# sadPororo/AD-YOLO

Measured on AMD Instinct MI355X. Metric: train-step audio-sec/s (4ch, se-resnet34+adyolo), higher is better.
Workload: dtype f32

## Files before the change

### ad-yolo_amd/_lib.py

```python
import ctypes
import os

_HERE = os.path.dirname(os.path.abspath(__file__))
LIB_PATH = os.environ.get("ADYOLO_LIB") or os.path.join(_HERE, "libadyolo_hip.so")

P = ctypes.c_void_p
I = ctypes.c_int
L = ctypes.c_long
F = ctypes.c_float
U64 = ctypes.c_uint64

SIGNATURES = {
    "adyolo_abi_version": (I, []),
    "adyolo_last_error": (ctypes.c_char_p, []),
    "adyolo_feat_stft_mel": (I, [P] * 8 + [I, I] + [P] * 4 + [I, I, I, P]),
    "adyolo_feat_finish": (I, [P] * 4 + [I, I, I, P]),
    "adyolo_feat_gcc_phat": (I, [P] * 6 + [I, I, I, I, P]),
    "adyolo_nchw_to_nhwc8": (I, [P, P, I, I, I, I, P]),
    "adyolo_pack_w3x3": (I, [P, P, P, I, I, I, P]),
    "adyolo_conv3x3_tiles": (I, [I] * 3),
    "adyolo_conv3x3_fwd": (I, [P] * 13 + [I] * 7 + [P]),
    "adyolo_wino_pack_w": (I, [P, P, P, I, I, I, P]),
    "adyolo_wino_pack_many": (I, [P, I, I, I, P]),
    "adyolo_wino_tiles": (I, [I] * 3),
    "adyolo_wino_fwd": (I, [P] * 13 + [I] * 7 + [P]),
    "adyolo_wino4_pack_w": (I, [P, P, P, I, I, I, P]),
    "adyolo_wino4_pack_many": (I, [P, I, I, I, P]),
    "adyolo_wino4_tiles": (I, [I] * 3),
    "adyolo_wino4_fwd": (I, [P] * 13 + [I] * 7 + [P]),
    "adyolo_wino4_last_form": (I, []),
    "adyolo_reload_switches": (I, []),
    "adyolo_wino4_wgrad_slabs": (I, [I] * 5),
    "adyolo_wino4_wgrad": (I, [P] * 7 + [I] * 6 + [P]),
    "adyolo_wino_wgrad_slabs": (I, [I] * 5),
    "adyolo_wino_wgrad": (I, [P] * 7 + [I] * 6 + [P]),
    "adyolo_conv3x3_wgrad_slabs": (I, [I] * 5),
    "adyolo_conv3x3_wgrad": (I, [P] * 6 + [I] * 6 + [P]),
    "adyolo_gemm": (I, [P] * 5 + [I] * 10 + [P]),
    "adyolo_gemm_batched": (I, [P] * 3 + [I] * 10 + [L] * 6 + [F, I, P]),
    "adyolo_colsum": (I, [P, P, P, I, I, I, I, P]),
    "adyolo_bn_stats": (I, [P] * 7 + [I, I, I, F, F, P]),
    "adyolo_bn_stats_tiles": (I, [P] * 11 + [I, I, I, I, F, F, P]),
    "adyolo_bn_eval_stats": (I, [P] * 4 + [I, F, P]),
    "adyolo_bn_scale_shift": (I, [P] * 6 + [I, P]),
    "adyolo_affine_nhwc": (I, [P] * 4 + [L, I, P]),
    "adyolo_bn_bwd_reduce": (I, [P] * 7 + [L, I, P]),
    "adyolo_bn_bwd_tiles": (I, [P, P, P, P, I, I, P]),
    "adyolo_bn_bwd_apply": (I, [P] * 12 + [L, I, I, F, P]),
# ... 120 lines not shown
```

### ad-yolo_amd/csrc/common.hpp

```cpp
#pragma once
#include <hip/hip_runtime.h>
#include <stdint.h>
#include <stdio.h>
#include "../../include/adyolo_hip.h"

typedef float f32x16 __attribute__((ext_vector_type(16)));
typedef float f32x4 __attribute__((ext_vector_type(4)));

namespace adyolo {

void set_error(const char *fmt, ...);

inline hipStream_t as_stream(void *s) { return reinterpret_cast<hipStream_t>(s); }

inline int check_launch(const char *what) {
    hipError_t e = hipGetLastError();
    if (e != hipSuccess) {
        set_error("%s: %s", what, hipGetErrorString(e));
        return (int)e;
    }
    return 0;
}

#define ADYOLO_REQUIRE(cond, code, ...)      \
// ... 26 lines not shown

__device__ __forceinline__ void mask_bits4(const unsigned long long *__restrict__ mask, size_t i, bool &x, bool &y,
                                           bool &z, bool &w) {
    const ulonglong2 lo = *reinterpret_cast<const ulonglong2 *>(mask + (i >> 6) * 4);
    const ulonglong2 hi = *reinterpret_cast<const ulonglong2 *>(mask + (i >> 6) * 4 + 2);
    const int b = (int)(i & 63);
    x = (lo.x >> b) & 1ull; y = (lo.y >> b) & 1ull; z = (hi.x >> b) & 1ull; w = (hi.y >> b) & 1ull;
}

__device__ __forceinline__ bool mask_bit1(const unsigned long long *__restrict__ mask, size_t o) {
    const size_t i = o >> 2;
    return (mask[(i >> 6) * 4 + (o & 3)] >> (i & 63)) & 1ull;
}

__device__ __forceinline__ float sigmoidf_(float x) { return 1.0f / (1.0f + expf(-x)); }

__device__ __forceinline__ double block_colsum32(const float *__restrict__ partial, int nparts, size_t ld, int c0,
                                                 int C, double *red) {
    const int cx = threadIdx.x & 31, py = threadIdx.x >> 5;
    const int c = c0 + cx;
    double s = 0.0;
    if (c < C) {
        double s1 = 0.0, s2 = 0.0, s3 = 0.0;
        int p = py;
        for (; p + 24 < nparts; p += 32) {
            const float a0 = partial[(size_t)p * ld + c], a1 = partial[(size_t)(p + 8) * ld + c];
            const float a2 = partial[(size_t)(p + 16) * ld + c], a3 = partial[(size_t)(p + 24) * ld + c];
            s += (double)a0;
            s1 += (double)a1;
            s2 += (double)a2;
// ... 55 lines not shown
```

### ad-yolo_amd/csrc/norm.hip

```cpp
#include "common.hpp"

namespace adyolo {

#ifndef ADYOLO_EW_NT
#define ADYOLO_EW_NT 3
#endif
__device__ __forceinline__ float4 ew_ld(const float4 *p) {
#if ADYOLO_EW_NT & 1
    const f32x4 v = __builtin_nontemporal_load(reinterpret_cast<const f32x4 *>(p));
    return make_float4(v[0], v[1], v[2], v[3]);
#else
    return *p;
#endif
}
__device__ __forceinline__ void ew_st(float4 *p, const float4 &v) {
#if ADYOLO_EW_NT & 2
    const f32x4 t = {v.x, v.y, v.z, v.w};
    __builtin_nontemporal_store(t, reinterpret_cast<f32x4 *>(p));
#else
    *p = v;
#endif
}


// ... 183 lines not shown

#ifndef ADYOLO_EW_U
#define ADYOLO_EW_U 4
#endif
constexpr int EW_U = ADYOLO_EW_U;


template <bool INV>
__global__ __launch_bounds__(256) void bn_bwd_apply_kernel(
    const float *__restrict__ dy, const float *__restrict__ x, const float *__restrict__ gamma,
    const float *__restrict__ mean, const float *__restrict__ invstd, const float *__restrict__ sdy,
    const float *__restrict__ sdyx, float *__restrict__ dx, float *__restrict__ sum_partial, long n4, int c4n, float invR,
    int relu_mask) {
    __shared__ float4 sred[256];
    float4 sacc = make_float4(0.f, 0.f, 0.f, 0.f);
    float4 g, m, is, a, b;
    auto load_params = [&](int cx) {
        g = reinterpret_cast<const float4 *>(gamma)[cx];
        m = reinterpret_cast<const float4 *>(mean)[cx];
        is = reinterpret_cast<const float4 *>(invstd)[cx];
        a = reinterpret_cast<const float4 *>(sdy)[cx];
        b = reinterpret_cast<const float4 *>(sdyx)[cx];
    };
    auto one = [&](float4 d, float4 xv) {
        float4 o;
        o.x = g.x * is.x * (d.x - a.x * invR - (xv.x - m.x) * is.x * b.x * invR);
        o.y = g.y * is.y * (d.y - a.y * invR - (xv.y - m.y) * is.y * b.y * invR);
        o.z = g.z * is.z * (d.z - a.z * invR - (xv.z - m.z) * is.z * b.z * invR);
        o.w = g.w * is.w * (d.w - a.w * invR - (xv.w - m.w) * is.w * b.w * invR);
        if (relu_mask) {
            if (!(xv.x > 0.f)) o.x = 0.f;
            if (!(xv.y > 0.f)) o.y = 0.f;
            if (!(xv.z > 0.f)) o.z = 0.f;
            if (!(xv.w > 0.f)) o.w = 0.f;
        }
        sacc.x += o.x; sacc.y += o.y; sacc.z += o.z; sacc.w += o.w;
        return o;
    };
    const float4 *dy4 = reinterpret_cast<const float4 *>(dy), *x4 = reinterpret_cast<const float4 *>(x);
    float4 *dx4 = reinterpret_cast<float4 *>(dx);
    if (INV) {
        load_params((int)threadIdx.x % c4n);
        const long step = (long)gridDim.x * 256 * EW_U;
        for (long i0 = (long)blockIdx.x * 256 * EW_U + threadIdx.x; i0 < n4; i0 += step) {
            float4 d[EW_U], xv[EW_U];
#pragma unroll
            for (int u = 0; u < EW_U; ++u) {
                const long i = i0 + u * 256;
                if (i < n4) {
                    d[u] = ew_ld(&dy4[i]);
// ... 736 lines not shown
```

### ad-yolo_amd/csrc/wino4w.hip

```cpp
#include "wino4_common.hpp"

namespace adyolo {
namespace w4 {

#ifndef W4W_WHATIF
#define W4W_WHATIF 0
#endif
#ifndef W4W_LD_AUX
#define W4W_LD_AUX 0
#endif
#ifndef W4W_TIMING
#define W4W_TIMING 0
#endif

__device__ __forceinline__ void a6v(const f32x4 (&v)[4], f32x4 (&t)[6]) {
    auto fm = [](float k, f32x4 a, f32x4 b) { return pkfma4(k, a, b); };
    const f32x4 z = {0.f, 0.f, 0.f, 0.f};
    const f32x4 ea = fm(A2, v[2], v[0]), oa = fm(A3, v[3], fm(PA, v[1], z));
    const f32x4 eb = fm(B2, v[2], v[0]), ob = fm(B3, v[3], fm(PB, v[1], z));
    t[0] = v[0];
    t[1] = ea + oa;
    t[2] = fm(-1.f, oa, ea);
    t[3] = eb + ob;
    t[4] = fm(-1.f, ob, eb);
// ... 12 lines not shown
#if W4W_TIMING
__device__ unsigned long long *g_w4w_stamps;
#endif

constexpr int XROWB = 1024;
constexpr int XSLOTS = 10;
constexpr int XNU = XSLOTS * XROWB;
constexpr int XBYTES = 6 * XNU;
template <int NB>
struct DCfg {
    static constexpr int DROWB = 1024 * NB;
    static constexpr int DNU = 4 * DROWB;
    static constexpr int DBUF = 6 * DNU;
};

template <bool AFF, int NB>
__global__ __launch_bounds__(256, 1) void wino4_wgrad_kernel(
    const float *__restrict__ x, const float *__restrict__ dy, const float *__restrict__ in_scale,
    const float *__restrict__ in_shift, float *__restrict__ slabs, int N, int H, int W, int Cin, int Cout, int runsW, int npairs,
    int nseg, int seg_steps, int nitems, int nsplit, int ciBlocks, int nblk) {
    constexpr int DROWB = DCfg<NB>::DROWB, DNU = DCfg<NB>::DNU, DBUF = DCfg<NB>::DBUF;
    constexpr int XOFF = 2 * DBUF;
    __shared__ __attribute__((aligned(16))) float lds[(XBYTES + 2 * DBUF) / 4 + (AFF ? 64 : 0)];
    char *ldsb = reinterpret_cast<char *>(lds);
    constexpr int AFFOFF = XBYTES + 2 * DBUF;

    const int tid = threadIdx.x, lane = tid & 63;
    const int wave = __builtin_amdgcn_readfirstlane(tid >> 6);
    const int li = lane & 31, lh = lane >> 5;
#if W4W_TIMING
    unsigned long long *stamps = g_w4w_stamps;
    int tstep = 0;
    auto tstamp = [&](int k) {
        if (blockIdx.x == 8 && tid == 0 && tstep < 12) stamps[tstep * 16 + k] = __builtin_amdgcn_s_memtime();
    };
#else
    auto tstamp = [&](int) {};
#endif
    int split, blk;
    if (32 % nblk == 0 && (int)gridDim.x == 8 * 32) {
// ... 20 lines not shown
    f32x16 acc[9][NB];
#pragma unroll
    for (int s = 0; s < 9; ++s)
#pragma unroll
        for (int cb = 0; cb < NB; ++cb)
#pragma unroll
            for (int r = 0; r < 16; ++r) acc[s][cb][r] = 0.f;

    const int run = wave & 1;
    const int sxr = (wave >> 1) * 2 + lh, sdr = sxr;
    const int st = li >> 3, sq = li & 7;
    if (AFF) {
        if (tid < 32) lds[AFFOFF / 4 + tid] = in_scale[c0 + tid];
        else if (tid < 64) lds[AFFOFF / 4 + tid] = in_shift[c0 + tid - 32];
    }
    const int xrowb = W * Cin * 4, drowb = W * Cout * 4, xpixb = Cin * 4, dpixb = Cout * 4;
    const __amdgpu_buffer_rsrc_t xrs = __builtin_amdgcn_make_buffer_rsrc(const_cast<float *>(x), 0, (int)((size_t)N * H * W * Cin * 4), 0x00020000);
    const __amdgpu_buffer_rsrc_t drs = __builtin_amdgcn_make_buffer_rsrc(const_cast<float *>(dy), 0, (int)((size_t)N * H * W * Cout * 4), 0x00020000);
    int wl[4];
#pragma unroll
    for (int k = 0; k < 4; ++k) wl[k] = (4 * sq + ((k + sq) & 3)) * 32 + ((run ^ ((sq >> 1) & 1)) << 4) + st * 4;

    for (int item = split; item < nitems; item += nsplit) {
        const int seg = item % nseg;
        const int pair = item / nseg;
        const int q = 2 * pair + run;
        const int tW = runsW < 0 ? -runsW : 0;
        bool qok, offL, offR;
        int n, col0;
        if (tW) {
            const int sh = tW == 1 ? 0 : 1;
            n = q * (4 >> sh) + (st >> sh);
            const int tcol = st & (tW - 1);
// ... 43 lines not shown
#pragma unroll
                for (int i = 1; i < 5; ++i) xpx[i] = pkfma4v(xpx[i], xsc, shv);
                xpx[5] = pkfma4v(xpx[5], xsc, offR ? zero : shv);
            }
            bt6v(xpx);
        };
        int wx[4];
        auto x_wr2 = [&](int nu) {
#pragma unroll
            for (int k = 0; k < 4; ++k) {
                *reinterpret_cast<float *>(ldsb + wx[k] + nu * XNU) = xpx[nu][k];
                *reinterpret_cast<float *>(ldsb + wx[k] + (nu + 1) * XNU) = xpx[nu + 1][k];
            }
        };
        f32x4 dpx[NB][4], de, dq;
        const int dlane = qok ? (int)(dbase + (unsigned)sdr * (unsigned)drowb) : (int)0x80000000;
        auto d_load = [&](int trow, int cb0 = 0, int cb1 = NB, int i0 = 0, int i1 = 4) {
            const int srow = __builtin_amdgcn_readfirstlane(4 * trow * drowb);
#pragma unroll
            for (int cb = cb0; cb < cb1; ++cb)
#pragma unroll
                for (int i = i0; i < i1; ++i)
                    dpx[cb][i] = __builtin_bit_cast(f32x4, __builtin_amdgcn_raw_buffer_load_b128(drs, dlane, srow + cb * 128 + i * dpixb, W4W_LD_AUX));
        };
        int wd[4];
        auto d_put2 = [&](int cb, int nu, const f32x4 &v, const f32x4 &v1) {
#pragma unroll
            for (int k = 0; k < 4; ++k) {
                *reinterpret_cast<float *>(ldsb + wd[k] + cb * 1024 + nu * DNU) = v[k];
                *reinterpret_cast<float *>(ldsb + wd[k] + cb * 1024 + (nu + 1) * DNU) = v1[k];
            }
        };
        auto d_part = [&](int cb, int part) {
            auto fm = [](float k, f32x4 a_, f32x4 b_) { return pkfma4(k, a_, b_); };
            const f32x4 z = {0.f, 0.f, 0.f, 0.f};
            const f32x4(&v)[4] = dpx[cb];
            if (part == 0) {
                de = fm(A2, v[2], v[0]);
// ... 17 lines not shown
        for (int k = 0; k < 4; ++k) wx[k] = wl[k] + XOFF + sxr * XROWB;
#pragma unroll
        for (int nu = 0; nu < 6; nu += 2) x_wr2(nu);
        if (sxr < 2) {
            x_load(4 * t0 + 3 + sxr);
            x_prep(4 * t0 + 3 + sxr);
#pragma unroll
            for (int k = 0; k < 4; ++k) wx[k] = wl[k] + XOFF + (4 + sxr) * XROWB;
#pragma unroll
            for (int nu = 0; nu < 6; nu += 2) x_wr2(nu);
        }
#pragma unroll
        for (int k = 0; k < 4; ++k) wd[k] = wl[k] + sdr * DROWB;
#pragma unroll
        for (int cb = 0; cb < NB; ++cb) {
            d_part(cb, 0);
            d_part(cb, 1);
            d_part(cb, 2);
        }
        x_load(4 * (t0 + 1) + 1 + sxr);
        d_load(t0 + 1);
        __syncthreads();

        f32x4 a[9], b[9];
        f32x4 vF[4], vH[4], zH;
        f32x4 cF[6], cP[4], cZ[3];
        auto d_reads_full = [&](int buf_, int cb) {
            const char *dp = ldsb + buf_ * DBUF + cb * 1024 + lx;
#pragma unroll
            for (int i = 0; i < 4; ++i) vF[i] = *reinterpret_cast<const f32x4 *>(dp + nuF * DNU + i * DROWB);
// ... 52 lines not shown
            d_reads_half(buf_, 0);
        };
        auto top_xform = [&]() {
            bt6v2(cF, a[0], a[1], a[2], a[3], a[4], a[5]);
            d_xform_full();
        };
        top_full(std::integral_constant<int, 0>{}, 0);
        top_half(std::integral_constant<int, 0>{}, 0);
        top_xform();
        auto step = [&](auto ROT_, int k) {
            constexpr int rot = decltype(ROT_)::value;
            constexpr std::integral_constant<int, (rot + 4) % XSLOTS> rotn{};
            asm volatile("" : "+s"(k));
            const int buf = k & 1;
            const int gyn = 4 * (t0 + k + 1) + 1 + sxr;
            auto side = [&](int t) {
                const int gy2 = 4 * (t0 + k + 2) + 1 + sxr, tr2 = min(t0 + k + 2, H / 4 - 1);
                if (t == 1) {
                    bt3v(cP, cZ, a[6], a[7], a[8], K2x, KPx);
                    d_xform_half();
                }
                if (NB == 2) {
                    if ((W4W_WHATIF & 2) && t != 1 && t != 8 && t != 10 && t < 14) return;
                    if (t == 2) x_prep(gyn);
                    if (t >= 3 && t <= 5) x_wr2(2 * (t - 3));
                    if (t >= 4 && t <= 6) x_load(gy2, 2 * (t - 4), 2 * (t - 4) + 2);
                    if (t >= 6 && t <= 8) d_part(0, t - 6);
                    if (t == 8) {
                        d_reads_full(buf, 1);
                        d_reads_half(buf, 1);
                    }
                    if (t == 9) d_load(tr2, 0, 1, 0, 2);
                    if (t == 10) {
                        d_xform_half();
                        d_load(tr2, 0, 1, 2, 4);
                    }
                    if (t >= 11 && t <= 13) d_part(1, t - 11);
                    if (t == 14) __syncthreads();
                    if (t == 15) {
                        top_full(rotn, buf ^ 1);
                        d_load(tr2, 1, 2, 0, 2);
                    }
                    if (t == 16) {
                        top_xform();
                        d_load(tr2, 1, 2, 2, 4);
                    }
                    if (t == 17) top_half(rotn, buf ^ 1);
                } else {
                    if (t == 0) x_prep(gyn);
                    if (t >= 1 && t <= 3) x_wr2(2 * (t - 1));
                    if (t >= 2 && t <= 4) x_load(gy2, 2 * (t - 2), 2 * (t - 2) + 2);
                    if (t >= 3 && t <= 5) d_part(0, t - 3);
                    if (t == 5) d_load(tr2);
                    if (t == 6) {
                        __syncthreads();
                        top_full(rotn, buf ^ 1);
                    }
                    if (t == 7) top_xform();
                    if (t == 8) top_half(rotn, buf ^ 1);
                }
            };
            tstamp(0);
            {
                constexpr int base = (rot + 6) % XSLOTS;
                const int soff = ((base + 2 >= XSLOTS && wave >= 2) ? (base - XSLOTS) * XROWB : base * XROWB) + XOFF + sxr * XROWB;
#pragma unroll
// ... 142 lines not shown
using namespace adyolo;

#if W4W_TIMING
extern "C" int adyolo_w4w_timing_buffer(void *p) {
    return hipMemcpyToSymbol(HIP_SYMBOL(w4::g_w4w_stamps), &p, sizeof(p)) == hipSuccess ? 0 : -1;
}
#endif

extern "C" int adyolo_wino4_wgrad_slabs(int N, int H, int W, int Cin, int Cout) {
    if (N <= 0 || H <= 0 || W <= 0 || Cin <= 0 || Cout <= 0) return ADYOLO_EINVAL;
    if (Cin % 32 || Cout % 32 || (W % 16 && W != 4 && W != 8) || H % 4 || H < 8) return 0;
    if ((size_t)N * H * W * (size_t)(Cin > Cout ? Cin : Cout) * 4 >= ((size_t)1 << 31)) return 0;
    return w4::wino4_wgrad_geometry(N, H, W, Cin, Cout, nullptr, nullptr, nullptr, nullptr, nullptr);
}

extern "C" int adyolo_wino4_wgrad(const float *x, const float *dy, const float *in_scale, const float *in_shift, float *slabs,
                                  float *du, float *dw, int N, int H, int W, int Cin, int Cin_real, int Cout, void *stream) {
    ADYOLO_REQUIRE(x && dy && slabs && du && dw && N > 0 && H > 0 && W > 0, ADYOLO_EINVAL, "wino4_wgrad: bad arguments");
    ADYOLO_REQUIRE(adyolo_wino4_wgrad_slabs(N, H, W, Cin, Cout) > 0 && Cin_real > 0 && Cin_real <= Cin, ADYOLO_ENOSUP,
                   "wino4_wgrad: unsupported shape N=%d H=%d W=%d Cin=%d Cout=%d (needs Cin %% 32 == 0, Cout %% 32 == 0, W %% 16 == 0 or W = 4 | 8, "
                   "H %% 4 == 0, tensors below 2 GiB)", N, H, W, Cin, Cout);
    ADYOLO_REQUIRE((in_scale == nullptr) == (in_shift == nullptr), ADYOLO_EINVAL, "wino4_wgrad: in_scale/in_shift come together");
    ADYOLO_REQUIRE(((reinterpret_cast<size_t>(x) | reinterpret_cast<size_t>(dy) | reinterpret_cast<size_t>(in_scale) |
                     reinterpret_cast<size_t>(in_shift)) & 15) == 0, ADYOLO_ENOSUP, "wino4_wgrad: x, dy, in_scale, in_shift must be 16-byte aligned");
    hipStream_t st = as_stream(stream);
    int npairs, nseg, seg_steps, nitems, nblk;
    const int nsplit = w4::wino4_wgrad_geometry(N, H, W, Cin, Cout, &npairs, &nseg, &seg_steps, &nitems, &nblk);
    const unsigned grid = (unsigned)(nsplit * nblk);
#define ADYOLO_W4W(AFF_, NB_)                                                                                          \
    hipLaunchKernelGGL((w4::wino4_wgrad_kernel<AFF_, NB_>), dim3(grid), dim3(256), 0, st, x, dy, in_scale, in_shift, slabs, N, H, \
                       W, Cin, Cout, W >= 16 ? W / 16 : -(W / 4), npairs, nseg, seg_steps, nitems, nsplit, Cin / 32, nblk)
    if (Cout % 64 == 0) {
        if (in_scale) ADYOLO_W4W(true, 2); else ADYOLO_W4W(false, 2);
    } else {
        if (in_scale) ADYOLO_W4W(true, 1); else ADYOLO_W4W(false, 1);
    }
#undef ADYOLO_W4W
    int rc = check_launch("wino4_wgrad");
    if (rc) return rc;
    hipLaunchKernelGGL(w4::wino4_wgrad_reduce_kernel, dim3(cdiv(Cin * Cout, 32), 36), dim3(256), 0, st, slabs, du, nsplit, Cin * Cout);
    rc = check_launch("wino4_wgrad_reduce");
    if (rc) return rc;
    hipLaunchKernelGGL(w4::wino4_wgrad_finish_kernel, dim3(cdiv(Cin * Cout, 256)), dim3(256), 0, st, du, dw, Cin, Cin_real, Cout);
    return check_launch("wino4_wgrad_finish");
}
```

### ad-yolo_amd/functional.py

```python
import os
from typing import NamedTuple

import torch

from . import ops

FUSE_BNBWD = os.environ.get("ADYOLO_FUSE_BNBWD", "1") != "0"
FUSE_POOL = os.environ.get("ADYOLO_FUSE_POOL", "1") != "0"
FUSE_POOL_BWD = os.environ.get("ADYOLO_FUSE_POOL_BWD", "1") != "0"


class BlockLink:

    def __init__(self):
        self.cc = self.mean2 = self.invstd2 = self.tiles = self.ebits = None
        self.affine = self.stem_bn = None
        self.prepooled = None


class BlockArgs(NamedTuple):
    bn1: object
    bn2: object
    bnd: object = None
    link_in: object = None
# ... 299 lines not shown
        vg1, vb1 = SINK.view(pg1), SINK.view(pb1)
        sunk = vse is not None and vw1 is not None and vw2 is not None and vg1 is not None and vb1 is not None
        if not sunk:
            vse = vw1 = vw2 = vg1 = vb1 = None
        de_full = None
        if pooled_hw is not None and not ctx.has_down:
            de_full = torch.empty(n, pooled_hw[0], pooled_hw[1], c, dtype=torch.float32, device=de.device)
        dc, dr, dg2, db2, dfw1, dfb1, dfw2, dfb2 = ops.se_tail_bwd(de, e, cc, g2, b2, mean2, invstd2, ssum2, pooled,
                                                                   hid, s, fw1, fw2,
                                                                   want_dr=ctx.has_down, tile_stats=tiles,
                                                                   mask=ebits, packed_out=vse, pooled_hw=pooled_hw,
                                                                   de_out=de_full)
        if pooled_hw is not None:
            de = de_full
        dw2 = ops.conv3x3_wgrad(a, dc, c, in_affine=(scale1, shift1), out=vw2)
        if FUSE_BNBWD:
            dbb, st = ops.conv3x3(dc, wpk2d, c, want_stats=True, stat_bn=(a, mean1, invstd1))
            da, dg1, db1 = ops.bn_bwd(dbb, a, g1, mean1, invstd1, relu_mask=True, tile_stats=st, out_dgamma=vg1,
                                      out_dbeta=vb1)
        else:
            dbb = ops.conv3x3(dc, wpk2d, c)
            da, dg1, db1 = ops.bn_bwd(dbb, a, g1, mean1, invstd1, relu_mask=True, out_dgamma=vg1, out_dbeta=vb1)
        dw1 = ops.conv3x3_wgrad(p, da, cin, in_affine=ctx.p_aff, out=vw1)
        if sunk:
            SINK.done(*pse)
            SINK.done(pw2, pg1, pb1, pw1)
            dw1 = dg1 = db1 = dw2 = dg2 = db2 = dfw1 = dfb1 = dfw2 = dfb2 = None
        dwd = dgd = dbd = None
        if ctx.has_down:
            q, wd, gd, meand, invstdd = t[20:25]
            pwd, pgd, pbd, wdshape = ctx.down_ptrs
            vwd, vgd, vbd = SINK.view(pwd, (wdshape[0], wdshape[1])), SINK.view(pgd), SINK.view(pbd)
            dsunk = sunk and vwd is not None and vgd is not None and vbd is not None
            if not dsunk:
                vwd = vgd = vbd = None
            dq, dgd, dbd = ops.bn_bwd(dr, q, gd, meand, invstdd, relu_mask=False, out_dgamma=vgd, out_dbeta=vbd)
            rows = n * h * w_
            dwd = ops.gemm(dq, p, c, cin, rows, c, cin, trans_a=True, trans_b=True,
# ... 535 lines not shown
```

### ad-yolo_amd/ops.py

```python
import ctypes
import os

import numpy as np
import torch

from . import _lib

_c = _lib.call
NULL = ctypes.c_void_p(0)


def _p(t):
    if t is None:
        return NULL
    return ctypes.c_void_p(t.data_ptr())


def _stream():
    return ctypes.c_void_p(torch.cuda.current_stream().cuda_stream)


def _chk(*ts):
    for t in ts:
        if t is None:
# ... 102 lines not shown

W4_THRESHOLDS = {}
_THRESHOLD_KEYS = ("min_k", "min_k_addend", "min_wgs", "min_wgrad_work", "min_k_32")


def reload_thresholds():
    env = os.environ.get
    W4_THRESHOLDS.update(min_k=int(env("ADYOLO_W4_MIN_K", "32")),
                         min_k_addend=int(env("ADYOLO_W4_MIN_K_ADDEND", "32")),
                         min_wgs=int(env("ADYOLO_W4_MIN_WGS", "200")),
                         min_wgrad_work=int(env("ADYOLO_W4W_MIN_WORK", "6000000")),
                         min_k_32=int(env("ADYOLO_W4_MIN_K_32", "32")),
                         persist=env("ADYOLO_W4_PERSIST", "1") != "0",
                         narrow=env("ADYOLO_W4_NARROW", "1") != "0",
                         wino1d=env("ADYOLO_WINO1D", "1") != "0",
                         wgrad_algo=(env("ADYOLO_WGRAD_ALGO") or "").lower() or None)
    if _lib.loaded():
        _lib.load().adyolo_reload_switches()
    return {k: W4_THRESHOLDS[k] for k in _THRESHOLD_KEYS}


def switch_table():
    t = dict(W4_THRESHOLDS)
    t["conv_algo"] = conv_algo()
    return t


def switch_stamp():
    return tuple(sorted((k, str(v)) for k, v in switch_table().items()))


# ... 151 lines not shown
    return (y, stats) if want_stats else y


def wgrad_form(cin, cout, algo=None, shape=None):
    algo = algo or W4_THRESHOLDS["wgrad_algo"] or conv_algo()
    if algo == "winograd4" and shape is not None and cin % 32 == 0 and cout % 32 == 0:
        n, h, w = shape
        if (w % 16 == 0 or w in (4, 8)) and h % 4 == 0 and n * w // 16 * (h // 4) * cin * cout >= W4_THRESHOLDS["min_wgrad_work"] and \
                _lib.load().adyolo_wino4_wgrad_slabs(n, h, w, cin, cout) > 0:
            return "wino4_wgrad_kernel", 9.0 / 36.0
    if algo in ("winograd", "winograd4") and cin % 32 == 0 and cout % 32 == 0:
        return "wino_wgrad_kernel", 16.0 / 36.0
    return "conv3x3_wgrad_kernel", 1.0


def conv3x3_wgrad(x, dy, cin_real, in_affine=None, algo=None, out=None):
    _chk(x, dy)
    n, h, w, cin = x.shape
    cout = dy.shape[3]
    sc, sh = in_affine if in_affine is not None else (None, None)
    dw = out if out is not None else _new(x, cout, cin_real, 3, 3)
    form = wgrad_form(cin, cout, algo, (n, h, w))[0]
    if DISPATCH_LOG is not None:
        k = (form, cin, cout, 1 if in_affine is not None else 0)
        DISPATCH_LOG[k] = DISPATCH_LOG.get(k, 0) + 1
    if form == "wino4_wgrad_kernel":
        nslab = _lib.load().adyolo_wino4_wgrad_slabs(n, h, w, cin, cout)
        slabs = _new(x, nslab, 36, cin, cout)
        du = _new(x, 36, cin, cout)
        _c("adyolo_wino4_wgrad", _p(x), _p(dy), _p(sc), _p(sh), _p(slabs), _p(du), _p(dw), n, h, w, cin, cin_real, cout, _stream())
# ... 140 lines not shown


def affine(x, scale, shift):
    _chk(x, scale, shift)
    c = x.shape[-1]
    y = torch.empty_like(x)
    _c("adyolo_affine_nhwc", _p(x), _p(scale), _p(shift), _p(y), x.numel() // c, c, _stream())
    return y


def bn_bwd(dy, x, gamma, mean, invstd, relu_mask=False, tile_stats=None, out_dgamma=None, out_dbeta=None,
           want_dx_colsum=False):
    _chk(dy, x, gamma, mean, invstd)
    c = x.shape[-1]
    rows = x.numel() // c
    sdy = out_dbeta if out_dbeta is not None else _new(x, c)
    sdyx = out_dgamma if out_dgamma is not None else _new(x, c)
    if tile_stats is not None:
        _c("adyolo_bn_bwd_tiles", _p(tile_stats), _p(sdy), _p(sdyx), _p(_new(tile_stats, 2, 256, c)), tile_stats.shape[1], c,
           _stream())
    else:
        partial = _new(x, 2 * 1024 * c)
        _c("adyolo_bn_bwd_reduce", _p(dy), _p(x), _p(mean), _p(invstd), _p(sdy), _p(sdyx), _p(partial), rows, c,
           _stream())
    dx = torch.empty_like(x)
    colsum = part = None
    if want_dx_colsum:
        colsum, part = _new(x, c), _new(x, 8192, c)
    a_sdy, a_sdyx, cs = sdy, sdyx, 1.0
    if EXACT.on:
        glob = EXACT.all_reduce(torch.stack([sdy, sdyx]))
        a_sdy, a_sdyx, cs = glob[0], glob[1], float(EXACT.world)
    _c("adyolo_bn_bwd_apply", _p(dy), _p(x), _p(gamma), _p(mean), _p(invstd), _p(a_sdy), _p(a_sdyx), _p(dx), NULL, NULL,
       _p(colsum), _p(part), rows, c, int(relu_mask), cs, _stream())
    if want_dx_colsum:
        return dx, sdyx, sdy, colsum
    return dx, sdyx, sdy


def se_fc_fwd(ssum, scale, shift, w1, b1, w2, b2, hw):
    _chk(ssum, scale, shift, w1, b1, w2, b2)
    n, c = ssum.shape
    cr = w1.shape[0]
    pooled, hid, s = _new(ssum, n, c), _new(ssum, n, cr), _new(ssum, n, c)
    _c("adyolo_se_fc_fwd", _p(ssum), _p(scale), _p(shift), _p(w1), _p(b1), _p(w2), _p(b2), _p(pooled), _p(hid), _p(s),
       n, hw, c, cr, _stream())
    return pooled, hid, s
# ... 656 lines not shown
```

### include/adyolo_hip.h

```cpp
#ifndef ADYOLO_HIP_H
#define ADYOLO_HIP_H

#include <stddef.h>
#include <stdint.h>

#ifdef __cplusplus
extern "C" {
#endif

#define ADYOLO_ABI_VERSION 1
#define ADYOLO_EINVAL (-1)
#define ADYOLO_ENOSUP (-2)

int         adyolo_abi_version(void);
const char *adyolo_last_error(void);

int adyolo_feat_stft_mel(const float *audio, const int64_t *clip_offset, const float *twiddle,
                         const int32_t *chunk_mel, const int32_t *chunk_start, const int32_t *chunk_len,
                         const int32_t *chunk_off, const float *mel_w, int n_chunks, int n_mel_w,
                         const float *scaler_mean, const float *scaler_rstd, float *out, float *chan_max, int B,
                         int n_samples, int layout, void *stream);
int adyolo_feat_finish(float *out, const float *chan_max, const float *scaler_mean,
                       const float *scaler_rstd, int B, int T, int layout, void *stream);

// ... 20 lines not shown
                    int N, int H, int W, int Cin, int Cout, int relu, int mask_bits, void *stream);
int adyolo_wino4_pack_w(const float *w , float *u_fwd , float *u_dgrad ,
                        int Cout, int Cin_real, int Cin, void *stream);
int adyolo_wino4_pack_many(const int64_t *table, int n, int max_cout, int max_cin, void *stream);
int adyolo_wino4_tiles(int N, int H, int W);
int adyolo_wino4_fwd(const float *x, const float *u, const float *bias, const float *addend, const float *addend_mask,
                     const float *in_scale, const float *in_shift, float *y, float *stats, const float *stat_aux,
                     const float *stat_mean, const float *stat_invstd, const float *stat_mask, int N, int H, int W, int Cin,
                     int Cout, int relu, int mask_bits, void *stream);
int adyolo_wino4_last_form(void);
int adyolo_reload_switches(void);
int adyolo_wino4_wgrad_slabs(int N, int H, int W, int Cin, int Cout);
int adyolo_wino4_wgrad(const float *x, const float *dy, const float *in_scale , const float *in_shift ,
                       float *slabs, float *du , float *dw, int N, int H, int W, int Cin, int Cin_real,
                       int Cout, void *stream);
int adyolo_wino_wgrad_slabs(int N, int H, int W, int Cin, int Cout);
int adyolo_wino_wgrad(const float *x, const float *dy, const float *in_scale, const float *in_shift, float *slabs,
                      float *du, float *dw, int N, int H, int W, int Cin, int Cin_real, int Cout, void *stream);
int adyolo_conv3x3_wgrad_slabs(int N, int H, int W, int Cin, int Cout);
int adyolo_conv3x3_wgrad(const float *x, const float *dy, const float *in_scale, const float *in_shift,
                         float *slabs, float *dw, int N, int H, int W, int Cin, int Cin_real, int Cout,
                         void *stream);

int adyolo_gemm(const float *A, const float *B, const float *bias, float *C, float *slabs, int M,
                int N, int K, int lda, int ldb, int ldc, int transA, int transB, int splits,
                int accumulate, void *stream);
int adyolo_gemm_batched(const float *A, const float *B, float *C, int M, int N, int K, int lda, int ldb, int ldc,
                        int transA, int transB, int outer, int inner, long oA, long iA, long oB, long iB, long oC,
                        long iC, float alpha, int accumulate, void *stream);
int adyolo_colsum(const float *A, float *out, float *partial, int R, int C, int lda, int accumulate,
// ... 197 lines not shown
```

Measured before the change: 36570.

## Fold BatchNorm backward apply into Winograd F4 weight-gradient kernel

For SE-ResNet blocks whose output channel count is not a multiple of 64, the BN1 backward apply (dx = k1*(dy - k2 - t*invR) with ReLU mask) now runs inside the wino4 weight-gradient kernel as it loads dy tiles. The kernel writes dx out from the first input-channel block, so the separate bn_bwd_apply pass and its re-read of dy and x go away. In exchange the wgrad kernel does an extra load of the BN input per tile, more LDS, and per-tile fold math. Shared BN coefficient math moves into a common helper with fp contraction turned off so both paths give the same numbers.

```diff
diff --git a/ad-yolo_amd/_lib.py b/ad-yolo_amd/_lib.py
--- a/ad-yolo_amd/_lib.py
+++ b/ad-yolo_amd/_lib.py
@@ -32,6 +32,7 @@
     "adyolo_reload_switches": (I, []),
     "adyolo_wino4_wgrad_slabs": (I, [I] * 5),
     "adyolo_wino4_wgrad": (I, [P] * 7 + [I] * 6 + [P]),
+    "adyolo_wino4_wgrad_bn": (I, [P] * 8 + [F] + [P] * 6 + [I] * 6 + [P]),
     "adyolo_wino_wgrad_slabs": (I, [I] * 5),
     "adyolo_wino_wgrad": (I, [P] * 7 + [I] * 6 + [P]),
     "adyolo_conv3x3_wgrad_slabs": (I, [I] * 5),
diff --git a/ad-yolo_amd/csrc/common.hpp b/ad-yolo_amd/csrc/common.hpp
--- a/ad-yolo_amd/csrc/common.hpp
+++ b/ad-yolo_amd/csrc/common.hpp
@@ -64,6 +64,21 @@
 }
 
 __device__ __forceinline__ float sigmoidf_(float x) { return 1.0f / (1.0f + expf(-x)); }
+
+__device__ __forceinline__ float bn_bwd_elem(float dy, float x, float k1, float k2, float mean, float is, float sdyx, float invR,
+                                             bool relu) {
+#pragma clang fp contract(off)
+    const float t = (x - mean) * is * sdyx;
+    const float o = k1 * fmaf(-t, invR, dy - k2);
+    return (relu && !(x > 0.f)) ? 0.f : o;
+}
+__device__ __forceinline__ f32x4 bn_bwd_quad(f32x4 dy, f32x4 x, f32x4 k1, f32x4 k2, f32x4 mean, f32x4 is, f32x4 sdyx, float invR,
+                                             bool relu) {
+    f32x4 o;
+#pragma unroll
+    for (int k = 0; k < 4; ++k) o[k] = bn_bwd_elem(dy[k], x[k], k1[k], k2[k], mean[k], is[k], sdyx[k], invR, relu);
+    return o;
+}
 
 __device__ __forceinline__ double block_colsum32(const float *__restrict__ partial, int nparts, size_t ld, int c0,
                                                  int C, double *red) {
diff --git a/ad-yolo_amd/csrc/norm.hip b/ad-yolo_amd/csrc/norm.hip
--- a/ad-yolo_amd/csrc/norm.hip
+++ b/ad-yolo_amd/csrc/norm.hip
@@ -221,26 +221,18 @@
     int relu_mask) {
     __shared__ float4 sred[256];
     float4 sacc = make_float4(0.f, 0.f, 0.f, 0.f);
-    float4 g, m, is, a, b;
+    f32x4 k1, k2, m, is, b;
     auto load_params = [&](int cx) {
-        g = reinterpret_cast<const float4 *>(gamma)[cx];
-        m = reinterpret_cast<const float4 *>(mean)[cx];
-        is = reinterpret_cast<const float4 *>(invstd)[cx];
-        a = reinterpret_cast<const float4 *>(sdy)[cx];
-        b = reinterpret_cast<const float4 *>(sdyx)[cx];
+        const f32x4 g = reinterpret_cast<const f32x4 *>(gamma)[cx], a = reinterpret_cast<const f32x4 *>(sdy)[cx];
+        m = reinterpret_cast<const f32x4 *>(mean)[cx];
+        is = reinterpret_cast<const f32x4 *>(invstd)[cx];
+        b = reinterpret_cast<const f32x4 *>(sdyx)[cx];
+        k1 = g * is;
+        k2 = a * invR;
     };
     auto one = [&](float4 d, float4 xv) {
-        float4 o;
-        o.x = g.x * is.x * (d.x - a.x * invR - (xv.x - m.x) * is.x * b.x * invR);
-        o.y = g.y * is.y * (d.y - a.y * invR - (xv.y - m.y) * is.y * b.y * invR);
-        o.z = g.z * is.z * (d.z - a.z * invR - (xv.z - m.z) * is.z * b.z * invR);
-        o.w = g.w * is.w * (d.w - a.w * invR - (xv.w - m.w) * is.w * b.w * invR);
-        if (relu_mask) {
-            if (!(xv.x > 0.f)) o.x = 0.f;
-            if (!(xv.y > 0.f)) o.y = 0.f;
-            if (!(xv.z > 0.f)) o.z = 0.f;
-            if (!(xv.w > 0.f)) o.w = 0.f;
-        }
+        const f32x4 r = bn_bwd_quad(f32x4{d.x, d.y, d.z, d.w}, f32x4{xv.x, xv.y, xv.z, xv.w}, k1, k2, m, is, b, invR, relu_mask != 0);
+        const float4 o = make_float4(r[0], r[1], r[2], r[3]);
         sacc.x += o.x; sacc.y += o.y; sacc.z += o.z; sacc.w += o.w;
         return o;
     };
diff --git a/ad-yolo_amd/csrc/wino4w.hip b/ad-yolo_amd/csrc/wino4w.hip
--- a/ad-yolo_amd/csrc/wino4w.hip
+++ b/ad-yolo_amd/csrc/wino4w.hip
@@ -50,16 +50,23 @@
     static constexpr int DBUF = 6 * DNU;
 };
 
-template <bool AFF, int NB>
+struct BnFold {
+    const float *x, *gamma, *mean, *invstd, *sdy, *sdyx;
+    float *dy_out;
+    float invR;
+};
+
+template <bool AFF, int NB, bool BNB = false>
 __global__ __launch_bounds__(256, 1) void wino4_wgrad_kernel(
     const float *__restrict__ x, const float *__restrict__ dy, const float *__restrict__ in_scale,
     const float *__restrict__ in_shift, float *__restrict__ slabs, int N, int H, int W, int Cin, int Cout, int runsW, int npairs,
-    int nseg, int seg_steps, int nitems, int nsplit, int ciBlocks, int nblk) {
+    int nseg, int seg_steps, int nitems, int nsplit, int ciBlocks, int nblk, BnFold bnf = {}) {
     constexpr int DROWB = DCfg<NB>::DROWB, DNU = DCfg<NB>::DNU, DBUF = DCfg<NB>::DBUF;
     constexpr int XOFF = 2 * DBUF;
-    __shared__ __attribute__((aligned(16))) float lds[(XBYTES + 2 * DBUF) / 4 + (AFF ? 64 : 0)];
+    __shared__ __attribute__((aligned(16))) float lds[(XBYTES + 2 * DBUF) / 4 + (AFF ? 64 : 0) + (BNB ? 5 * 32 * NB : 0)];
     char *ldsb = reinterpret_cast<char *>(lds);
     constexpr int AFFOFF = XBYTES + 2 * DBUF;
+    constexpr int BNOFF = AFFOFF + (AFF ? 256 : 0);
 
     const int tid = threadIdx.x, lane = tid & 63;
     const int wave = __builtin_amdgcn_readfirstlane(tid >> 6);
@@ -110,9 +117,21 @@
         if (tid < 32) lds[AFFOFF / 4 + tid] = in_scale[c0 + tid];
         else if (tid < 64) lds[AFFOFF / 4 + tid] = in_shift[c0 + tid - 32];
     }
+    if (BNB && tid < 32 * NB) {
+        const int c = co0 + tid;
+        const float is = bnf.invstd[c];
+        lds[BNOFF / 4 + tid] = bnf.gamma[c] * is;
+        lds[BNOFF / 4 + 32 * NB + tid] = bnf.sdy[c] * bnf.invR;
+        lds[BNOFF / 4 + 64 * NB + tid] = bnf.mean[c];
+        lds[BNOFF / 4 + 96 * NB + tid] = is;
+        lds[BNOFF / 4 + 128 * NB + tid] = bnf.sdyx[c];
+    }
     const int xrowb = W * Cin * 4, drowb = W * Cout * 4, xpixb = Cin * 4, dpixb = Cout * 4;
     const __amdgpu_buffer_rsrc_t xrs = __builtin_amdgcn_make_buffer_rsrc(const_cast<float *>(x), 0, (int)((size_t)N * H * W * Cin * 4), 0x00020000);
     const __amdgpu_buffer_rsrc_t drs = __builtin_amdgcn_make_buffer_rsrc(const_cast<float *>(dy), 0, (int)((size_t)N * H * W * Cout * 4), 0x00020000);
+    const __amdgpu_buffer_rsrc_t brs = __builtin_amdgcn_make_buffer_rsrc(const_cast<float *>(BNB ? bnf.x : dy), 0, (int)((size_t)N * H * W * Cout * 4), 0x00020000);
+    const __amdgpu_buffer_rsrc_t ors = __builtin_amdgcn_make_buffer_rsrc(BNB ? bnf.dy_out : nullptr, 0, (int)((size_t)N * H * W * Cout * 4), 0x00020000);
+    const bool bwr = BNB && ibk == 0;
     int wl[4];
 #pragma unroll
     for (int k = 0; k < 4; ++k) wl[k] = (4 * sq + ((k + sq) & 3)) * 32 + ((run ^ ((sq >> 1) & 1)) << 4) + st * 4;
@@ -186,14 +205,33 @@
             }
         };
         f32x4 dpx[NB][4], de, dq;
+        f32x4 bpx[BNB ? NB : 1][4];
         const int dlane = qok ? (int)(dbase + (unsigned)sdr * (unsigned)drowb) : (int)0x80000000;
         auto d_load = [&](int trow, int cb0 = 0, int cb1 = NB, int i0 = 0, int i1 = 4) {
             const int srow = __builtin_amdgcn_readfirstlane(4 * trow * drowb);
 #pragma unroll
             for (int cb = cb0; cb < cb1; ++cb)
 #pragma unroll
-                for (int i = i0; i < i1; ++i)
+                for (int i = i0; i < i1; ++i) {
                     dpx[cb][i] = __builtin_bit_cast(f32x4, __builtin_amdgcn_raw_buffer_load_b128(drs, dlane, srow + cb * 128 + i * dpixb, W4W_LD_AUX));
+                    if (BNB)
+                        bpx[cb][i] = __builtin_bit_cast(f32x4, __builtin_amdgcn_raw_buffer_load_b128(brs, dlane, srow + cb * 128 + i * dpixb, W4W_LD_AUX));
+                }
+        };
+        auto d_fold = [&](int cb, int trow, bool put) {
+            if (!BNB) return;
+            const int so = BNOFF + cb * 128 + (lane & 7) * 16;
+            const f32x4 k1 = *reinterpret_cast<const f32x4 *>(ldsb + so), k2 = *reinterpret_cast<const f32x4 *>(ldsb + so + 128 * NB);
+            const f32x4 mu = *reinterpret_cast<const f32x4 *>(ldsb + so + 256 * NB), is = *reinterpret_cast<const f32x4 *>(ldsb + so + 384 * NB);
+            const f32x4 sx = *reinterpret_cast<const f32x4 *>(ldsb + so + 512 * NB);
+#pragma unroll
+            for (int i = 0; i < 4; ++i) dpx[cb][i] = bn_bwd_quad(dpx[cb][i], bpx[cb][i], k1, k2, mu, is, sx, bnf.invR, true);
+            if (bwr && put) {
+                const int srow = __builtin_amdgcn_readfirstlane(4 * trow * drowb);
+#pragma unroll
+                for (int i = 0; i < 4; ++i)
+                    __builtin_amdgcn_raw_buffer_store_b128(__builtin_bit_cast(u32x4_t, dpx[cb][i]), ors, dlane, srow + cb * 128 + i * dpixb, 0);
+            }
         };
         int wd[4];
         auto d_put2 = [&](int cb, int nu, const f32x4 &v, const f32x4 &v1) {
@@ -241,6 +279,7 @@
         for (int k = 0; k < 4; ++k) wd[k] = wl[k] + sdr * DROWB;
 #pragma unroll
         for (int cb = 0; cb < NB; ++cb) {
+            d_fold(cb, t0, true);
             d_part(cb, 0);
             d_part(cb, 1);
             d_part(cb, 2);
@@ -323,6 +362,7 @@
             asm volatile("" : "+s"(k));
             const int buf = k & 1;
             const int gyn = 4 * (t0 + k + 1) + 1 + sxr;
+            const bool dput = k + 1 < nsteps;
             auto side = [&](int t) {
                 const int gy2 = 4 * (t0 + k + 2) + 1 + sxr, tr2 = min(t0 + k + 2, H / 4 - 1);
                 if (t == 1) {
@@ -334,6 +374,7 @@
                     if (t == 2) x_prep(gyn);
                     if (t >= 3 && t <= 5) x_wr2(2 * (t - 3));
                     if (t >= 4 && t <= 6) x_load(gy2, 2 * (t - 4), 2 * (t - 4) + 2);
+                    if (t == 6) d_fold(0, t0 + k + 1, dput);
                     if (t >= 6 && t <= 8) d_part(0, t - 6);
                     if (t == 8) {
                         d_reads_full(buf, 1);
@@ -344,6 +385,7 @@
                         d_xform_half();
                         d_load(tr2, 0, 1, 2, 4);
                     }
+                    if (t == 11) d_fold(1, t0 + k + 1, dput);
                     if (t >= 11 && t <= 13) d_part(1, t - 11);
                     if (t == 14) __syncthreads();
                     if (t == 15) {
@@ -359,6 +401,7 @@
                     if (t == 0) x_prep(gyn);
                     if (t >= 1 && t <= 3) x_wr2(2 * (t - 1));
                     if (t >= 2 && t <= 4) x_load(gy2, 2 * (t - 2), 2 * (t - 2) + 2);
+                    if (t == 3) d_fold(0, t0 + k + 1, dput);
                     if (t >= 3 && t <= 5) d_part(0, t - 3);
                     if (t == 5) d_load(tr2);
                     if (t == 6) {
@@ -531,8 +574,8 @@
     return w4::wino4_wgrad_geometry(N, H, W, Cin, Cout, nullptr, nullptr, nullptr, nullptr, nullptr);
 }
 
-extern "C" int adyolo_wino4_wgrad(const float *x, const float *dy, const float *in_scale, const float *in_shift, float *slabs,
-                                  float *du, float *dw, int N, int H, int W, int Cin, int Cin_real, int Cout, void *stream) {
+static int wino4_wgrad_launch(const float *x, const float *dy, const float *in_scale, const float *in_shift, float *slabs, float *du,
+                              float *dw, int N, int H, int W, int Cin, int Cin_real, int Cout, const w4::BnFold *bn, void *stream) {
     ADYOLO_REQUIRE(x && dy && slabs && du && dw && N > 0 && H > 0 && W > 0, ADYOLO_EINVAL, "wino4_wgrad: bad arguments");
     ADYOLO_REQUIRE(adyolo_wino4_wgrad_slabs(N, H, W, Cin, Cout) > 0 && Cin_real > 0 && Cin_real <= Cin, ADYOLO_ENOSUP,
                    "wino4_wgrad: unsupported shape N=%d H=%d W=%d Cin=%d Cout=%d (needs Cin %% 32 == 0, Cout %% 32 == 0, W %% 16 == 0 or W = 4 | 8, "
@@ -540,17 +583,25 @@
     ADYOLO_REQUIRE((in_scale == nullptr) == (in_shift == nullptr), ADYOLO_EINVAL, "wino4_wgrad: in_scale/in_shift come together");
     ADYOLO_REQUIRE(((reinterpret_cast<size_t>(x) | reinterpret_cast<size_t>(dy) | reinterpret_cast<size_t>(in_scale) |
                      reinterpret_cast<size_t>(in_shift)) & 15) == 0, ADYOLO_ENOSUP, "wino4_wgrad: x, dy, in_scale, in_shift must be 16-byte aligned");
+    ADYOLO_REQUIRE(!bn || Cout % 64 != 0, ADYOLO_ENOSUP, "wino4_wgrad_bn: only for Cout %% 64 != 0 (32-channel output blocks)");
+    if (bn)
+        ADYOLO_REQUIRE(bn->x && bn->gamma && bn->mean && bn->invstd && bn->sdy && bn->sdyx && bn->dy_out &&
+                           ((reinterpret_cast<size_t>(bn->x) | reinterpret_cast<size_t>(bn->dy_out)) & 15) == 0,
+                       ADYOLO_EINVAL, "wino4_wgrad_bn: bad BatchNorm operands (all needed; bn_x and dy_out 16-byte aligned)");
     hipStream_t st = as_stream(stream);
     int npairs, nseg, seg_steps, nitems, nblk;
     const int nsplit = w4::wino4_wgrad_geometry(N, H, W, Cin, Cout, &npairs, &nseg, &seg_steps, &nitems, &nblk);
     const unsigned grid = (unsigned)(nsplit * nblk);
-#define ADYOLO_W4W(AFF_, NB_)                                                                                          \
-    hipLaunchKernelGGL((w4::wino4_wgrad_kernel<AFF_, NB_>), dim3(grid), dim3(256), 0, st, x, dy, in_scale, in_shift, slabs, N, H, \
-                       W, Cin, Cout, W >= 16 ? W / 16 : -(W / 4), npairs, nseg, seg_steps, nitems, nsplit, Cin / 32, nblk)
-    if (Cout % 64 == 0) {
-        if (in_scale) ADYOLO_W4W(true, 2); else ADYOLO_W4W(false, 2);
+    const w4::BnFold bnf = bn ? *bn : w4::BnFold{};
+#define ADYOLO_W4W(AFF_, NB_, BNB_)                                                                                      \
+    hipLaunchKernelGGL((w4::wino4_wgrad_kernel<AFF_, NB_, BNB_>), dim3(grid), dim3(256), 0, st, x, dy, in_scale, in_shift, slabs, N, \
+                       H, W, Cin, Cout, W >= 16 ? W / 16 : -(W / 4), npairs, nseg, seg_steps, nitems, nsplit, Cin / 32, nblk, bnf)
+    if (bn) {
+        if (in_scale) ADYOLO_W4W(true, 1, true); else ADYOLO_W4W(false, 1, true);
+    } else if (Cout % 64 == 0) {
+        if (in_scale) ADYOLO_W4W(true, 2, false); else ADYOLO_W4W(false, 2, false);
     } else {
-        if (in_scale) ADYOLO_W4W(true, 1); else ADYOLO_W4W(false, 1);
+        if (in_scale) ADYOLO_W4W(true, 1, false); else ADYOLO_W4W(false, 1, false);
     }
 #undef ADYOLO_W4W
     int rc = check_launch("wino4_wgrad");
@@ -561,3 +612,19 @@
     hipLaunchKernelGGL(w4::wino4_wgrad_finish_kernel, dim3(cdiv(Cin * Cout, 256)), dim3(256), 0, st, du, dw, Cin, Cin_real, Cout);
     return check_launch("wino4_wgrad_finish");
 }
+
+extern "C" int adyolo_wino4_wgrad(const float *x, const float *dy, const float *in_scale, const float *in_shift, float *slabs,
+                                  float *du, float *dw, int N, int H, int W, int Cin, int Cin_real, int Cout, void *stream) {
+    return wino4_wgrad_launch(x, dy, in_scale, in_shift, slabs, du, dw, N, H, W, Cin, Cin_real, Cout, nullptr, stream);
+}
+
+extern "C" int adyolo_wino4_wgrad_bn(const float *x, const float *dbb, const float *bn_x, const float *gamma, const float *mean,
+                                     const float *invstd, const float *sdy, const float *sdyx, float count_scale, const float *in_scale,
+                                     const float *in_shift, float *slabs, float *du, float *dw, float *dx_out, int N, int H, int W,
+                                     int Cin, int Cin_real, int Cout, void *stream) {
+    ADYOLO_REQUIRE(count_scale >= 1.f, ADYOLO_EINVAL, "wino4_wgrad_bn: count_scale must be >= 1");
+    const long rows = (long)N * H * W;
+    const w4::BnFold bn{bn_x, gamma, mean, invstd, sdy, sdyx, dx_out,
+                        (float)(1.0 / ((double)rows * (double)count_scale))};
+    return wino4_wgrad_launch(x, dbb, in_scale, in_shift, slabs, du, dw, N, H, W, Cin, Cin_real, Cout, &bn, stream);
+}
diff --git a/ad-yolo_amd/functional.py b/ad-yolo_amd/functional.py
--- a/ad-yolo_amd/functional.py
+++ b/ad-yolo_amd/functional.py
@@ -337,14 +337,19 @@
         if pooled_hw is not None:
             de = de_full
         dw2 = ops.conv3x3_wgrad(a, dc, c, in_affine=(scale1, shift1), out=vw2)
-        if FUSE_BNBWD:
+        if FUSE_BNBWD and ops.wgrad_bn_fold_ok(cin, c, (n, h, w_)):
             dbb, st = ops.conv3x3(dc, wpk2d, c, want_stats=True, stat_bn=(a, mean1, invstd1))
-            da, dg1, db1 = ops.bn_bwd(dbb, a, g1, mean1, invstd1, relu_mask=True, tile_stats=st, out_dgamma=vg1,
-                                      out_dbeta=vb1)
-        else:
-            dbb = ops.conv3x3(dc, wpk2d, c)
-            da, dg1, db1 = ops.bn_bwd(dbb, a, g1, mean1, invstd1, relu_mask=True, out_dgamma=vg1, out_dbeta=vb1)
-        dw1 = ops.conv3x3_wgrad(p, da, cin, in_affine=ctx.p_aff, out=vw1)
+            da, dg1, db1, dw1 = ops.conv3x3_wgrad_bn(p, dbb, cin, a, g1, mean1, invstd1, st, in_affine=ctx.p_aff, out=vw1,
+                                                     out_dgamma=vg1, out_dbeta=vb1)
+        else:
+            if FUSE_BNBWD:
+                dbb, st = ops.conv3x3(dc, wpk2d, c, want_stats=True, stat_bn=(a, mean1, invstd1))
+                da, dg1, db1 = ops.bn_bwd(dbb, a, g1, mean1, invstd1, relu_mask=True, tile_stats=st, out_dgamma=vg1,
+                                          out_dbeta=vb1)
+            else:
+                dbb = ops.conv3x3(dc, wpk2d, c)
+                da, dg1, db1 = ops.bn_bwd(dbb, a, g1, mean1, invstd1, relu_mask=True, out_dgamma=vg1, out_dbeta=vb1)
+            dw1 = ops.conv3x3_wgrad(p, da, cin, in_affine=ctx.p_aff, out=vw1)
         if sunk:
             SINK.done(*pse)
             SINK.done(pw2, pg1, pb1, pw1)
diff --git a/ad-yolo_amd/ops.py b/ad-yolo_amd/ops.py
--- a/ad-yolo_amd/ops.py
+++ b/ad-yolo_amd/ops.py
@@ -140,7 +140,8 @@
                          persist=env("ADYOLO_W4_PERSIST", "1") != "0",
                          narrow=env("ADYOLO_W4_NARROW", "1") != "0",
                          wino1d=env("ADYOLO_WINO1D", "1") != "0",
-                         wgrad_algo=(env("ADYOLO_WGRAD_ALGO") or "").lower() or None)
+                         wgrad_algo=(env("ADYOLO_WGRAD_ALGO") or "").lower() or None,
+                         fuse_bn1_bwd=env("ADYOLO_FUSE_BN1_BWD", "1") != "0")
     if _lib.loaded():
         _lib.load().adyolo_reload_switches()
     return {k: W4_THRESHOLDS[k] for k in _THRESHOLD_KEYS}
@@ -322,6 +323,48 @@
     return "conv3x3_wgrad_kernel", 1.0
 
 
+def wgrad_bn_fold_ok(cin, cout, shape):
+    return (W4_THRESHOLDS["fuse_bn1_bwd"] and cout % 64 != 0 and
+            wgrad_form(cin, cout, shape=shape)[0] == "wino4_wgrad_kernel")
+
+
+def bn_bwd_sums(dy, x, tile_stats=None, mean=None, invstd=None, out_dgamma=None, out_dbeta=None):
+    c = x.shape[-1]
+    sdy = out_dbeta if out_dbeta is not None else _new(x, c)
+    sdyx = out_dgamma if out_dgamma is not None else _new(x, c)
+    if tile_stats is not None:
+        _c("adyolo_bn_bwd_tiles", _p(tile_stats), _p(sdy), _p(sdyx), _p(_new(tile_stats, 2, 256, c)), tile_stats.shape[1], c,
+           _stream())
+    else:
+        partial = _new(x, 2 * 1024 * c)
+        _c("adyolo_bn_bwd_reduce", _p(dy), _p(x), _p(mean), _p(invstd), _p(sdy), _p(sdyx), _p(partial), x.numel() // c, c,
+           _stream())
+    if EXACT.on:
+        glob = EXACT.all_reduce(torch.stack([sdy, sdyx]))
+        return sdy, sdyx, glob[0], glob[1], float(EXACT.world)
+    return sdy, sdyx, sdy, sdyx, 1.0
+
+
+def conv3x3_wgrad_bn(x, dbb, cin_real, bn_x, gamma, mean, invstd, tile_stats, in_affine=None, out=None, out_dgamma=None,
+                     out_dbeta=None):
+    _chk(x, dbb, bn_x, gamma, mean, invstd, tile_stats)
+    n, h, w, cin = x.shape
+    cout = dbb.shape[3]
+    sdy, sdyx, a_sdy, a_sdyx, cs = bn_bwd_sums(dbb, bn_x, tile_stats, out_dgamma=out_dgamma, out_dbeta=out_dbeta)
+    sc, sh = in_affine if in_affine is not None else (None, None)
+    dw = out if out is not None else _new(x, cout, cin_real, 3, 3)
+    da = torch.empty_like(bn_x)
+    if DISPATCH_LOG is not None:
+        k = ("wino4_wgrad_kernel", cin, cout, (1 if in_affine is not None else 0) | 2)
+        DISPATCH_LOG[k] = DISPATCH_LOG.get(k, 0) + 1
+    nslab = _lib.load().adyolo_wino4_wgrad_slabs(n, h, w, cin, cout)
+    slabs = _new(x, nslab, 36, cin, cout)
+    du = _new(x, 36, cin, cout)
+    _c("adyolo_wino4_wgrad_bn", _p(x), _p(dbb), _p(bn_x), _p(gamma), _p(mean), _p(invstd), _p(a_sdy), _p(a_sdyx), cs, _p(sc), _p(sh),
+       _p(slabs), _p(du), _p(dw), _p(da), n, h, w, cin, cin_real, cout, _stream())
+    return da, sdyx, sdy, dw
+
+
 def conv3x3_wgrad(x, dy, cin_real, in_affine=None, algo=None, out=None):
     _chk(x, dy)
     n, h, w, cin = x.shape
@@ -492,23 +535,11 @@
     _chk(dy, x, gamma, mean, invstd)
     c = x.shape[-1]
     rows = x.numel() // c
-    sdy = out_dbeta if out_dbeta is not None else _new(x, c)
-    sdyx = out_dgamma if out_dgamma is not None else _new(x, c)
-    if tile_stats is not None:
-        _c("adyolo_bn_bwd_tiles", _p(tile_stats), _p(sdy), _p(sdyx), _p(_new(tile_stats, 2, 256, c)), tile_stats.shape[1], c,
-           _stream())
-    else:
-        partial = _new(x, 2 * 1024 * c)
-        _c("adyolo_bn_bwd_reduce", _p(dy), _p(x), _p(mean), _p(invstd), _p(sdy), _p(sdyx), _p(partial), rows, c,
-           _stream())
+    sdy, sdyx, a_sdy, a_sdyx, cs = bn_bwd_sums(dy, x, tile_stats, mean, invstd, out_dgamma=out_dgamma, out_dbeta=out_dbeta)
     dx = torch.empty_like(x)
     colsum = part = None
     if want_dx_colsum:
         colsum, part = _new(x, c), _new(x, 8192, c)
-    a_sdy, a_sdyx, cs = sdy, sdyx, 1.0
-    if EXACT.on:
-        glob = EXACT.all_reduce(torch.stack([sdy, sdyx]))
-        a_sdy, a_sdyx, cs = glob[0], glob[1], float(EXACT.world)
     _c("adyolo_bn_bwd_apply", _p(dy), _p(x), _p(gamma), _p(mean), _p(invstd), _p(a_sdy), _p(a_sdyx), _p(dx), NULL, NULL,
        _p(colsum), _p(part), rows, c, int(relu_mask), cs, _stream())
     if want_dx_colsum:
diff --git a/include/adyolo_hip.h b/include/adyolo_hip.h
--- a/include/adyolo_hip.h
+++ b/include/adyolo_hip.h
@@ -58,6 +58,10 @@
 int adyolo_wino4_wgrad(const float *x, const float *dy, const float *in_scale , const float *in_shift ,
                        float *slabs, float *du , float *dw, int N, int H, int W, int Cin, int Cin_real,
                        int Cout, void *stream);
+int adyolo_wino4_wgrad_bn(const float *x, const float *dbb, const float *bn_x, const float *gamma, const float *mean,
+                          const float *invstd, const float *sdy, const float *sdyx, float count_scale, const float *in_scale ,
+                          const float *in_shift , float *slabs, float *du, float *dw, float *dx_out, int N, int H, int W,
+                          int Cin, int Cin_real, int Cout, void *stream);
 int adyolo_wino_wgrad_slabs(int N, int H, int W, int Cin, int Cout);
 int adyolo_wino_wgrad(const float *x, const float *dy, const float *in_scale, const float *in_shift, float *slabs,
                       float *du, float *dw, int N, int H, int W, int Cin, int Cin_real, int Cout, void *stream);
```

New measurement: 36750, median of 6. Within noise of the previous version (+0.5%).
